# kv13arm/mujoco_rl_manipulate_unknown_objects

Hardware: AMD Instinct MI355X
Metric: env-steps/sec (whole node), acorn_env 4096 envs/GPU (higher is better)
Workload: dtype f32

## Files before the change

### mujoco_rl_manipulate_unknown_objects_amd/csrc/grip_render.hip

```cpp
#include <hip/hip_runtime.h>
#include <cstdio>
#include <cstdlib>
#include <algorithm>
#include "grip_device.h"
#include <atomic>

int grip_fail(const char *msg);
static int launch_status(const char *what) {
    hipError_t e = hipGetLastError();
    if (e == hipSuccess) return 0;
    char buf[256]; snprintf(buf, sizeof buf, "%s: %s", what, hipGetErrorString(e));
    return grip_fail(buf);
}

#define RW 64
#define RH 64
#define RTHREADS 1024
#define RPIX (RW * RH)

struct Frames { float p[6][3]; float R[6][9]; float cam_o[3]; float cam_R[9]; };

__device__ static void compute_frames(const DevModel &m, const float *qpos, int n, int e, int half, Frames &f) {
    float q[14];
    for (int i = 0; i < 14; i++) q[i] = ld_word(qpos, (size_t)i * n + e, half);
    V3 pe = v3(m.ee_pos0[0] + q[0], m.ee_pos0[1] + q[1], m.ee_pos0[2] + q[2]);
    float sr = sinf(q[3]), cr = cosf(q[3]), sy = sinf(q[4]), cy = cosf(q[4]);
    M3 Re;
    Re.m[0] = cy; Re.m[1] = -sy; Re.m[2] = 0.f; Re.m[3] = cr * sy; Re.m[4] = cr * cy; Re.m[5] = -sr; Re.m[6] = sr * sy; Re.m[7] = sr * cy; Re.m[8] = cr;
    auto put = [&](int g, V3 p, const M3 &R) { f.p[g][0] = p.x; f.p[g][1] = p.y; f.p[g][2] = p.z; for (int i = 0; i < 9; i++) f.R[g][i] = R.m[i]; };
    V3 pb = pe + mulv(Re, ldv(m.base_pos)); M3 Rb = mulm(Re, ldm(m.base_R));
    put(0, pb, Rb);
    for (int s = 0; s < 2; s++) {
        V3 pk = pb + mulv(Rb, ldv(m.kn_pos[s])); M3 Rk0 = mulm(Rb, ldm(m.kn_R[s]));
        float sq = sinf(q[5 + s]), cq = cosf(q[5 + s]);
        M3 Ry; Ry.m[0] = cq; Ry.m[1] = 0; Ry.m[2] = sq; Ry.m[3] = 0; Ry.m[4] = 1; Ry.m[5] = 0; Ry.m[6] = -sq; Ry.m[7] = 0; Ry.m[8] = cq;
        M3 Rk = mulm(Rk0, Ry);
        put(1 + 2 * s, pk, Rk);
        put(2 + 2 * s, pk + mulv(Rk, ldv(m.fin_pos[s])), mulm(Rk, ldm(m.fin_R[s])));
    }
    float qn = rsqrtf(q[10] * q[10] + q[11] * q[11] + q[12] * q[12] + q[13] * q[13]);
    put(5, v3(q[7], q[8], q[9]), quat_mat(q[10] * qn, q[11] * qn, q[12] * qn, q[13] * qn));
    V3 co = pe + mulv(Re, ldv(m.cam_pos)); M3 Rc = mulm(Re, ldm(m.cam_R));
    f.cam_o[0] = co.x; f.cam_o[1] = co.y; f.cam_o[2] = co.z;
    for (int i = 0; i < 9; i++) f.cam_R[i] = Rc.m[i];
}


__device__ __forceinline__ void frame_role(const DevModel &m, const float *qpos, int n, int e, int half, int role, Frames &f) {
    auto Q = [&](int i) { return ld_word(qpos, (size_t)i * n + e, half); };
    V3 P; M3 R;
    if (role == 5) {
        const float q0 = Q(10), q1 = Q(11), q2 = Q(12), q3 = Q(13);
        const float qn = rsqrtf(q0 * q0 + q1 * q1 + q2 * q2 + q3 * q3);
        P = v3(Q(7), Q(8), Q(9)); R = quat_mat(q0 * qn, q1 * qn, q2 * qn, q3 * qn);
    } else {
        const V3 pe = v3(m.ee_pos0[0] + Q(0), m.ee_pos0[1] + Q(1), m.ee_pos0[2] + Q(2));
        const float q3 = Q(3), q4 = Q(4);
        const float sr = sinf(q3), cr = cosf(q3), sy = sinf(q4), cy = cosf(q4);
        M3 Re;
        Re.m[0] = cy; Re.m[1] = -sy; Re.m[2] = 0.f; Re.m[3] = cr * sy; Re.m[4] = cr * cy; Re.m[5] = -sr; Re.m[6] = sr * sy; Re.m[7] = sr * cy; Re.m[8] = cr;
        if (role == 6) { P = pe + mulv(Re, ldv(m.cam_pos)); R = mulm(Re, ldm(m.cam_R)); }
        else {
            P = pe + mulv(Re, ldv(m.base_pos)); R = mulm(Re, ldm(m.base_R));
            if (role >= 1) {
                const int s = role >= 3 ? 1 : 0;
                const V3 pk = P + mulv(R, ldv(m.kn_pos[s])); const M3 Rk0 = mulm(R, ldm(m.kn_R[s]));
                const float qk = Q(5 + s);
                const float sq = sinf(qk), cq = cosf(qk);
                M3 Ry; Ry.m[0] = cq; Ry.m[1] = 0; Ry.m[2] = sq; Ry.m[3] = 0; Ry.m[4] = 1; Ry.m[5] = 0; Ry.m[6] = -sq; Ry.m[7] = 0; Ry.m[8] = cq;
                P = pk; R = mulm(Rk0, Ry);
                if (role == 2 || role == 4) { const V3 pf = P + mulv(R, ldv(m.fin_pos[s])); const M3 Rf = mulm(R, ldm(m.fin_R[s])); P = pf; R = Rf; }
            }
        }
    }
    float *op = role == 6 ? f.cam_o : f.p[role], *oR = role == 6 ? f.cam_R : f.R[role];
    op[0] = P.x; op[1] = P.y; op[2] = P.z;
#pragma unroll
    for (int i = 0; i < 9; i++) oR[i] = R.m[i];
}

__device__ static uint8_t to_u8(float v) { v *= 255.f; v = fminf(fmaxf(v, 0.f), 255.f); return (uint8_t)v; }

__device__ __forceinline__ void lit_colour(const DevModel &m, int geom, float b0, float b1, float b2, V3 P, V3 N, V3 co, float &c0, float &c1, float &c2) {
    const float spec = m.geom_material[geom][0], shin = 128.f * m.geom_material[geom][1];
    const V3 V = normalized(co - P);
    float diff = m.geom_material[geom][2] + m.headlight[0], sp = 0.f;
    {   const float nv = dot(N, V);
        if (nv > 0.f) { diff += m.headlight[1] * nv; sp += m.headlight[2] * __powf(nv, shin); } }
#pragma unroll
    for (int l = 0; l < 2; l++) {
        const V3 ld = normalized(ldv(m.light_dir[l]));
        V3 L = -ld; float spot = 1.f;
        if (!m.light_directional[l]) {
            L = normalized(ldv(m.light_pos[l]) - P);
            const float c = -dot(L, ld);
            spot = c > m.light_params[l][3] ? __powf(c, m.light_params[l][4]) : 0.f;
        }
        diff += m.light_params[l][2];
        const float nl = dot(N, L);
        if (nl > 0.f && spot > 0.f) {
            diff += spot * m.light_params[l][0] * nl;
            const float nh = fmaxf(dot(N, normalized(L + V)), 0.f);
            sp += spot * m.light_params[l][1] * __powf(nh, shin);
        }
    }
    c0 = b0 * diff + spec * sp; c1 = b1 * diff + spec * sp; c2 = b2 * diff + spec * sp;
}
// ... 267 lines not shown
#pragma unroll
    for (int q = 0; q < TPX; q++) { float d = best[q] - dmin; if (d <= 1.0f) { lsum += d; lcnt++; } }
    red[tid] = lsum; redi[tid] = lcnt; __syncthreads();
    for (int s = RTHREADS / 2; s > 0; s >>= 1) { if (tid < s) { red[tid] += red[tid + s]; redi[tid] += redi[tid + s]; } __syncthreads(); }
    float scale = 2.0f * (red[0] / (float)redi[0]);
    if (cfg.full_observation) {
        unsigned db[TPX];
#pragma unroll
        for (int q = 0; q < TPX; q++) {
            float v = (best[q] - dmin) / scale; v = fminf(fmaxf(v, 0.f), 1.f);
            float p = 255.0f * v;
            db[q] = (p != p) ? 0u : (unsigned)(uint8_t)p;
        }
#pragma unroll
        for (int r = 0; r < TW; r++) put2(3, r, db[2 * r], db[2 * r + 1]);
    }
    __syncthreads();
    if (tid == 0) {
        const int pg_ = GPTR(const int, pad_grasp)[e], pp_ = GPTR(const int, pad_pher)[e];
        img[(nch - 1) * RPIX] = (uint8_t)pg_; img[(nch - 1) * RPIX + 1] = (uint8_t)pp_;
    }
    __syncthreads();
    const uint4 *src = reinterpret_cast<const uint4 *>(img);
    for (int i = tid; i < nch * RPIX / 16; i += RTHREADS) {
        const uint4 v = src[i];
        if (o) reinterpret_cast<uint4 *>(o)[i] = v;
        if (o2) reinterpret_cast<uint4 *>(o2)[i] = v;
    }
}

#ifndef RS_SMALL
#define RS_SMALL 16
#endif
#ifndef RS_WAVES
#define RS_WAVES 8
#endif
#ifndef RS_FACES
#define RS_FACES 255
#endif
#ifndef RS_QUAD
#define RS_QUAD 1
#endif
#define RS_LDS_BUDGET (80 * 1024 - 34 * 1024)
#define RS_DYN_BYTES(nverts, edges, items) ((size_t)(((nverts) * 3 + 3) / 4 * 4) * 4 + (size_t)RS_FACES * 32 + (size_t)(edges) * 16 + (size_t)(items) * 2)
struct __align__(16) RsFace { float4 P; int ebase, k, id, pad; };
static_assert(!RS_QUAD || RS_FACES <= 255, "a quad item holds the face record in 8 bits, and 0xffff must stay free");

__device__ __forceinline__ void rs_claim(unsigned long long *zb, int pix, float t, int id) {
    atomicMin(zb + pix, ((unsigned long long)__float_as_uint(t) << 32) | (unsigned)id);
}

__device__ __forceinline__ void observe_body_raster(const DevModel &m, const DevConfig &cfg, const float *qpos, const int *pad_grasp, const int *pad_pher,
                                                    int n, int e, uint8_t *obs, uint8_t *obs2, const long long *row2, int nverts_max, const int RS_EDGES, const int RS_ITEMS) {
    __shared__ Frames fr;
    __shared__ float gmx[GN_GEOM][12];
    __shared__ int gnum[GN_GEOM];
    __shared__ int nfaces, nedges, nitems;
    __shared__ __align__(16) unsigned char pool[8 * RPIX];
    extern __shared__ float4 rs_dyn[];
    unsigned long long *zb = reinterpret_cast<unsigned long long *>(pool);
    uint8_t *img = pool; float *red = reinterpret_cast<float *>(pool + 5 * RPIX); int *redi = reinterpret_cast<int *>(pool + 6 * RPIX);
    float *cv = reinterpret_cast<float *>(rs_dyn);
    RsFace *frec = reinterpret_cast<RsFace *>(cv + (nverts_max * 3 + 3) / 4 * 4);
    float4 *en = reinterpret_cast<float4 *>(frec + RS_FACES);
    unsigned short *items = reinterpret_cast<unsigned short *>(en + RS_EDGES);
    const int tid = threadIdx.x;
    const int nvert_all = m.hull_vadr[GN_HULL - 1] + m.hull_vnum[GN_HULL - 1], nplane_all = m.hull_padr[GN_HULL - 1] + m.hull_pnum[GN_HULL - 1];
    auto hull_of_vertex = [&](int i) { int g = 1; for (int h = 2; h < GN_GEOM; h++) g = i >= m.hull_vadr[h - 1] ? h : g; return g; };
    auto hull_of_plane = [&](int i) { int g = 1; for (int h = 2; h < GN_GEOM; h++) g = i >= m.hull_padr[h - 1] ? h : g; return g; };
    constexpr int VPT = 2;
    float4 vearly[VPT];
    {   const float4 *vb = reinterpret_cast<const float4 *>(m.hull_blob);
#pragma unroll
        for (int k = 0; k < VPT; k++) { const int i = tid + k * RTHREADS; vearly[k] = i < nvert_all ? vb[i] : make_float4(0.f, 0.f, 0.f, 0.f); }
    }
    if (tid < 7) frame_role(m, qpos, n, e, cfg.state_half, tid, fr);
    if (tid == 0) { nfaces = 0; nedges = 0; nitems = 0; }
    for (int i = tid; i < RPIX; i += RTHREADS) zb[i] = ~0ull;
    for (int i = tid; i < RS_ITEMS; i += RTHREADS) items[i] = 0xffffu;
    __syncthreads();
    if (tid >= 1 && tid < GN_GEOM) {
        const int g = tid;
        V3 co = ldv(fr.cam_o); M3 Rc = ldm(fr.cam_R);
        V3 p = ldv(fr.p[g - 1]); M3 R = ldm(fr.R[g - 1]);
        V3 c = multv(Rc, p + mulv(R, ldv(m.geom_center[g])) - co);
        float r = m.geom_rbound[g];
        M3 Mx = mulm(M3{{R.m[0], R.m[3], R.m[6], R.m[1], R.m[4], R.m[7], R.m[2], R.m[5], R.m[8]}}, Rc);
        V3 ol = multv(R, co - p);
#pragma unroll
        for (int i = 0; i < 9; i++) gmx[g][i] = Mx.m[i];
        gmx[g][9] = ol.x; gmx[g][10] = ol.y; gmx[g][11] = ol.z;
        bool vis = c.z - r < 0.f;
        if (vis) {
            const float th = tanf(0.5f * m.cam_fovy * 0.017453292519943295f) * 1.0001f;
            unsigned out = 0x1fu;
            for (int k = 0; k < 8; k++) {
                const V3 q = multv(Mx, v3(m.hull_aabb[g - 1][(k & 1) ? 3 : 0] - ol.x, m.hull_aabb[g - 1][(k & 2) ? 4 : 1] - ol.y, m.hull_aabb[g - 1][(k & 4) ? 5 : 2] - ol.z));
                const float d = -q.z * th + 1e-6f;
                unsigned o_ = 0u;
                o_ |= q.z > -m.znear ? 1u : 0u; o_ |= q.x > d ? 2u : 0u; o_ |= q.x < -d ? 4u : 0u; o_ |= q.y > d ? 8u : 0u; o_ |= q.y < -d ? 16u : 0u;
                out &= o_;
            }
            vis = out == 0u;
        }
        gnum[g] = vis ? m.hull_pnum[g - 1] : 0;
    }
    __syncthreads();
    const float tanh_ = tanf(0.5f * m.cam_fovy * 0.017453292519943295f);
    auto ray_x = [&](int px) { return (2.0f * (px + 0.5f) / RW - 1.0f) * tanh_; };
    auto ray_y = [&](int py) { return (1.0f - 2.0f * (py + 0.5f) / RH) * tanh_; };
    {
        const float4 *vb = reinterpret_cast<const float4 *>(m.hull_blob);
        auto to_camera = [&](int i, float4 v) {
            const int g = hull_of_vertex(i);
            const int *gn = gnum; asm volatile("" : "+v"(gn));
            if (!gn[g]) return;
            const M3 Mx = ldm(gmx[g]);
            const V3 c = multv(Mx, v3(v.x - gmx[g][9], v.y - gmx[g][10], v.z - gmx[g][11]));
            cv[3 * i] = c.x; cv[3 * i + 1] = c.y; cv[3 * i + 2] = c.z;
        };
#pragma unroll
        for (int k = 0; k < VPT; k++) if (tid + k * RTHREADS < nvert_all) to_camera(tid + k * RTHREADS, vearly[k]);
        for (int i = tid + VPT * RTHREADS; i < nvert_all; i += RTHREADS) to_camera(i, vb[i]);
    }
    __syncthreads();
#ifndef RS_STOP
#define RS_STOP 0
#endif
    if (RS_STOP != 1) {
        for (int i = tid; i < nplane_all; i += RTHREADS) {
            const int jg = nplane_all - 1 - i, g = hull_of_plane(jg), j = jg - m.hull_padr[g - 1];
            {   const int *gn = gnum; asm volatile("" : "+v"(gn)); if (!gn[g]) continue; }
            const int l0 = m.hull_ladr[jg], K = m.hull_ladr[jg + 1] - l0;
            if (K < 3) continue;
            const float *pl = m.hull_planes + 4 * jg;
            const V3 nn = v3(pl[0], pl[1], pl[2]);
            const M3 Mx = ldm(gmx[g]);
            const V3 A = multv(Mx, nn);
            const float B = pl[3] - dot(nn, v3(gmx[g][9], gmx[g][10], gmx[g][11]));
            if (!(B < 0.f)) continue;
            const float *cvg = cv + 3 * m.hull_vadr[g - 1];
            const int *lp = m.hull_loops + l0;
            int id4[4]; V3 v4[4];
            float xmin = 3.0e38f, xmax = -3.0e38f, ymin = 3.0e38f, ymax = -3.0e38f;
            const float zn = -m.znear;
            auto take = [&](float x, float y, float z) {
                const float iz = rcp(-z), px = x * iz, py = y * iz;
                xmin = fminf(xmin, px); xmax = fmaxf(xmax, px); ymin = fminf(ymin, py); ymax = fmaxf(ymax, py);
            };
            auto corner = [&](V3 prev, V3 cur) {
                const bool ic = cur.z <= zn, ip = prev.z <= zn;
                if (ic) take(cur.x, cur.y, cur.z);
                if (ic != ip) { const float s_ = (zn - prev.z) * rcp(cur.z - prev.z); take(fmaf(s_, cur.x - prev.x, prev.x), fmaf(s_, cur.y - prev.y, prev.y), zn); }
            };
            auto vert = [&](int id) { return v3(cvg[3 * id], cvg[3 * id + 1], cvg[3 * id + 2]); };
#pragma unroll
            for (int k = 0; k < 4; k++) { id4[k] = lp[k < K ? k : 0]; v4[k] = vert(id4[k]); }
            V3 prev = K == 3 ? v4[2] : (K == 4 ? v4[3] : vert(lp[K - 1]));
#pragma unroll
            for (int k = 0; k < 4; k++) if (k < K) { corner(prev, v4[k]); prev = v4[k]; }
            for (int k = 4; k < K; k++) { const V3 c = vert(lp[k]); corner(prev, c); prev = c; }
            if (!(xmin <= xmax)) continue;
            int x0, x1, y0, y1;
            {
                const float sx = 0.5f * RW / tanh_, sy = 0.5f * RH / tanh_;
                const float fx0 = xmin * sx + 0.5f * RW - 0.5f, fx1 = xmax * sx + 0.5f * RW - 0.5f;
                const float fy0 = 0.5f * RH - ymax * sy - 0.5f, fy1 = 0.5f * RH - ymin * sy - 0.5f;
                if (fx1 < -0.01f || fy1 < -0.01f || fx0 > RW - 0.99f || fy0 > RH - 0.99f) continue;
                x0 = (int)ceilf(fmaxf(fx0 - 0.01f, 0.f)); x1 = (int)floorf(fminf(fx1 + 0.01f, RW - 1.f));
                y0 = (int)ceilf(fmaxf(fy0 - 0.01f, 0.f)); y1 = (int)floorf(fminf(fy1 + 0.01f, RH - 1.f));
                if (x0 > x1 || y0 > y1) continue;
            }
            const int idw = (g << 16) | j;
            const int area = (x1 - x0 + 1) * (y1 - y0 + 1);
            auto edge = [&](int ia, V3 a, int ib, V3 b) { const bool sw = ia > ib; const V3 c = cross(sw ? b : a, sw ? a : b); return sw ? -c : c; };
            if (K <= 4 && area <= RS_SMALL) {
                V3 ne[4];
#pragma unroll
                for (int k = 0; k < 4; k++) {
                    const int kn = (k + 1 < K) ? k + 1 : 0;
                    ne[k] = k < K ? edge(id4[k], v4[k], id4[kn], v4[kn]) : v3(0.f, 0.f, 0.f);
                }
                int px = x0, py = y0;
                for (int q = 0; q < area; q++) {
                    const float x = ray_x(px), y = ray_y(py);
                    bool in = true;
#pragma unroll
                    for (int k = 0; k < 4; k++) in &= !(fmaf(ne[k].x, x, fmaf(ne[k].y, y, -ne[k].z)) > 0.f);
                    const float den = fmaf(A.y, y, fmaf(A.x, x, -A.z));
                    const float t = B * rcp(den);
                    if (in && den < 0.f && t > 0.f && t > m.znear) rs_claim(zb, py * RW + px, t, idw);
                    if (++px > x1) { px = x0; ++py; }
                }
                continue;
            }
            constexpr int TS = RS_QUAD ? 2 : 3, TB = RS_QUAD ? 8 : 6;
            const int tx0 = x0 >> TS, tx1 = x1 >> TS, ty0 = y0 >> TS, ty1 = y1 >> TS, ntile = (tx1 - tx0 + 1) * (ty1 - ty0 + 1);
            int fi = atomicAdd(&nfaces, 1), eb = -1, ib = -1;
            if (fi < RS_FACES) { eb = atomicAdd(&nedges, K); if (eb + K <= RS_EDGES) { ib = atomicAdd(&nitems, ntile); if (ib + ntile > RS_ITEMS) ib = -1; } }
            if (ib >= 0) {
                RsFace f; f.P = make_float4(A.x, A.y, A.z, B); f.ebase = eb; f.k = K; f.id = idw; f.pad = 0;
                frec[fi] = f;
                int ia = lp[0]; V3 a = v3(cvg[3 * ia], cvg[3 * ia + 1], cvg[3 * ia + 2]);
                const int i0 = ia; const V3 a0 = a;
                for (int k = 0; k < K; k++) {
                    const int ib2 = k + 1 < K ? lp[k + 1] : i0;
                    const V3 b = k + 1 < K ? v3(cvg[3 * ib2], cvg[3 * ib2 + 1], cvg[3 * ib2 + 2]) : a0;
                    const V3 c = edge(ia, a, ib2, b);
                    en[eb + k] = make_float4(c.x, c.y, c.z, 0.f);
                    ia = ib2; a = b;
                }
                int w = ib;
                for (int ty = ty0; ty <= ty1; ty++) for (int tx = tx0; tx <= tx1; tx++) items[w++] = (unsigned short)((fi << TB) | ((ty << (6 - TS)) + tx));
                continue;
            }
            for (int py = y0; py <= y1; py++) for (int px = x0; px <= x1; px++) {
                const float x = ray_x(px), y = ray_y(py);
                bool in = true;
                int ia = lp[0]; V3 a = v3(cvg[3 * ia], cvg[3 * ia + 1], cvg[3 * ia + 2]);
                const int i0 = ia; const V3 a0 = a;
                for (int k = 0; k < K; k++) {
                    const int ib2 = k + 1 < K ? lp[k + 1] : i0;
                    const V3 b = k + 1 < K ? v3(cvg[3 * ib2], cvg[3 * ib2 + 1], cvg[3 * ib2 + 2]) : a0;
                    const V3 c = edge(ia, a, ib2, b);
                    in &= !(fmaf(c.x, x, fmaf(c.y, y, -c.z)) > 0.f);
                    ia = ib2; a = b;
                }
                const float den = fmaf(A.y, y, fmaf(A.x, x, -A.z));
                const float t = B * rcp(den);
                if (in && den < 0.f && t > 0.f && t > m.znear) rs_claim(zb, py * RW + px, t, idw);
            }
        }
    }
    __syncthreads();
    if (RS_STOP != 1 && RS_STOP != 2) {
        const int ni = min(nitems, RS_ITEMS), wv = tid >> 6, ln = tid & 63;
#if RS_QUAD
        auto fetch = [&](int it0, unsigned &item, RsFace &f) {
            const int it = it0 + (ln >> 4);
            item = it < ni ? (unsigned)items[it] : 0xffffu;
            f = frec[item != 0xffffu ? (item >> 8) : 0];
        };
        unsigned item, item_n = 0xffffu; RsFace f, f_n;
        fetch(4 * wv, item, f);
        for (int it0 = 4 * wv; it0 < ni; it0 += 4 * (RTHREADS / 64)) {
            if (it0 + 4 * (RTHREADS / 64) < ni) fetch(it0 + 4 * (RTHREADS / 64), item_n, f_n);
            const bool live = item != 0xffffu;
            const int K = live ? f.k : 0;
            const int quad = item & 255, px = (quad & 15) * 4 + (ln & 3), py = (quad >> 4) * 4 + ((ln >> 2) & 3);
            const float x = ray_x(px), y = ray_y(py);
            bool in = live;
            const float4 *ep = en + f.ebase;
            for (int k0 = 0; __any(k0 < K); k0 += 4) {
                float4 c[4];
#pragma unroll
                for (int j = 0; j < 4; j++) c[j] = ep[max(min(k0 + j, K - 1), 0)];
#pragma unroll
                for (int j = 0; j < 4; j++) in &= !(fmaf(c[j].x, x, fmaf(c[j].y, y, -c[j].z)) > 0.f);
            }
            const float den = fmaf(f.P.y, y, fmaf(f.P.x, x, -f.P.z));
            const float t = f.P.w * rcp(den);
            if (in && den < 0.f && t > 0.f && t > m.znear) rs_claim(zb, py * RW + px, t, f.id);
            item = item_n; f = f_n; item_n = 0xffffu;
        }
#else
        for (int it = wv; it < ni; it += RTHREADS / 64) {
            const unsigned item = __builtin_amdgcn_readfirstlane((unsigned)items[it]);
            if (item == 0xffffu) continue;
            RsFace f = frec[item >> 6];
            f.k = __builtin_amdgcn_readfirstlane(f.k); f.ebase = __builtin_amdgcn_readfirstlane(f.ebase);
            const int tile = item & 63, px = (tile & 7) * 8 + (ln & 7), py = (tile >> 3) * 8 + (ln >> 3);
            const float x = ray_x(px), y = ray_y(py);
            bool in = true;
            const float4 *ep = en + f.ebase;
            for (int k = 0; k < f.k; k++) { const float4 c = ep[k]; in &= !(fmaf(c.x, x, fmaf(c.y, y, -c.z)) > 0.f); }
            const float den = fmaf(f.P.y, y, fmaf(f.P.x, x, -f.P.z));
            const float t = f.P.w * rcp(den);
            if (in && den < 0.f && t > 0.f && t > m.znear) rs_claim(zb, py * RW + px, t, f.id);
        }
#endif
    }
    __syncthreads();
    const Frames *frl = &fr;
    asm volatile("" : "+v"(frl));
    const int nch = cfg.full_observation ? 5 : 4;
    uint8_t *o = obs ? obs + (size_t)blockIdx.x * nch * RPIX : nullptr;
    uint8_t *o2 = obs2 ? obs2 + (size_t)(row2[0] + blockIdx.x) * nch * RPIX : nullptr;
    constexpr int WPR = RW / (8 * TW);
    const int w = tid >> 6, l = tid & 63;
    const int tx = (l & 7) + 8 * (w % WPR), ty = (l >> 3) + 8 * (w / WPR);
    float xs[TW], ys[TW];
#pragma unroll
    for (int a = 0; a < TW; a++) { xs[a] = ray_x(TW * tx + a); ys[a] = ray_y(TW * ty + a); }
    float best[TPX]; int hitent[TPX];
#pragma unroll
    for (int q = 0; q < TPX; q++) {
        float x = xs[q % TW], y = ys[q / TW];
        float dz = frl->cam_R[6] * x + frl->cam_R[7] * y - frl->cam_R[8];
        best[q] = m.zfar; hitent[q] = -1;
        if (dz < 0.f) { float t = -frl->cam_o[2] / dz; if (t > m.znear && t < best[q]) { best[q] = t; hitent[q] = 0; } }
        const unsigned long long z = zb[(TW * ty + q / TW) * RW + TW * tx + q % TW];
        const float th = __uint_as_float((unsigned)(z >> 32));
        if (z != ~0ull && th < best[q]) { best[q] = th; hitent[q] = (int)(unsigned)z; }
    }
    __syncthreads();
    asm volatile("" : "+v"(frl));
    const V3 co = ldv(frl->cam_o); const M3 Rc = ldm(frl->cam_R);
    float lmin = 3.0e38f;
#pragma unroll
    for (int q = 0; q < TPX; q++) {
        const float x = xs[q % TW], y = ys[q / TW];
        const V3 dir = mulv(Rc, v3(x, y, -1.f));
        const int hit = hitent[q] < 0 ? -1 : (hitent[q] >> 16);
        float c0, c1, c2;
        if (hit < 0) {
            V3 dn = normalized(dir); float f = 0.5f * (dn.z + 1.0f);
            c0 = m.sky_rgb[3] + f * (m.sky_rgb[0] - m.sky_rgb[3]); c1 = m.sky_rgb[4] + f * (m.sky_rgb[1] - m.sky_rgb[4]); c2 = m.sky_rgb[5] + f * (m.sky_rgb[2] - m.sky_rgb[5]);
        } else {
            float b0, b1, b2; V3 nrm = v3(0, 0, 1);
            const V3 Pw = co + dir * best[q];
            if (hit == 0) {
                int cx = (int)floorf(Pw.x * 8.0f), cy = (int)floorf(Pw.y * 8.0f);
                int off = ((cx + cy) & 1) ? 3 : 0;
                b0 = m.floor_rgb[off]; b1 = m.floor_rgb[off + 1]; b2 = m.floor_rgb[off + 2];
            } else {
                b0 = m.geom_rgba[hit][0]; b1 = m.geom_rgba[hit][1]; b2 = m.geom_rgba[hit][2];
                const float *pl = m.hull_planes + 4 * (m.hull_padr[hit - 1] + (hitent[q] & 0xffff));
                const V3 A = multv(ldm(gmx[hit]), v3(pl[0], pl[1], pl[2]));
                nrm = normalized(mulv(Rc, A));
            }
#if defined(RS_SKIP) && (RS_SKIP & 1)
            c0 = b0 * nrm.z; c1 = b1 * Pw.x; c2 = b2;
#else
            lit_colour(m, hit, b0, b1, b2, Pw, nrm, co, c0, c1, c2);
#endif
        }
        {   const int px = (TW * ty + q / TW) * RW + TW * tx + q % TW;
            img[px] = to_u8(c0); img[RPIX + px] = to_u8(c1); img[2 * RPIX + px] = to_u8(c2); }
        lmin = fminf(lmin, best[q]);
        __builtin_amdgcn_sched_barrier(0);
    }
    auto put2 = [&](int ch, int r, unsigned lo, unsigned hi) {
        const int px = (TW * ty + r) * RW + TW * tx;
        *reinterpret_cast<uint16_t *>(img + ch * RPIX + px) = (uint16_t)(lo | (hi << 8));
    };
#pragma unroll
    for (int r = 0; r < TW; r++) put2(nch - 1, r, 0u, 0u);
#if defined(RS_SKIP) && (RS_SKIP & 2)
    float dmin = lmin; red[0] = 1.f; redi[0] = 1;
#else
    red[tid] = lmin; __syncthreads();
    for (int s = RTHREADS / 2; s > 0; s >>= 1) { if (tid < s) red[tid] = fminf(red[tid], red[tid + s]); __syncthreads(); }
    float dmin = red[0]; __syncthreads();
    float lsum = 0.f; int lcnt = 0;
#pragma unroll
    for (int q = 0; q < TPX; q++) { float d = best[q] - dmin; if (d <= 1.0f) { lsum += d; lcnt++; } }
    red[tid] = lsum; redi[tid] = lcnt; __syncthreads();
    for (int s = RTHREADS / 2; s > 0; s >>= 1) { if (tid < s) { red[tid] += red[tid + s]; redi[tid] += redi[tid + s]; } __syncthreads(); }
#endif
    float scale = 2.0f * (red[0] / (float)redi[0]);
    if (cfg.full_observation) {
        unsigned db[TPX];
#pragma unroll
        for (int q = 0; q < TPX; q++) {
            float v = (best[q] - dmin) / scale; v = fminf(fmaxf(v, 0.f), 1.f);
            float p = 255.0f * v;
            db[q] = (p != p) ? 0u : (unsigned)(uint8_t)p;
        }
#pragma unroll
        for (int r = 0; r < TW; r++) put2(3, r, db[2 * r], db[2 * r + 1]);
    }
    __syncthreads();
    if (tid == 0) {
        const int pg_ = GPTR(const int, pad_grasp)[e], pp_ = GPTR(const int, pad_pher)[e];
        img[(nch - 1) * RPIX] = (uint8_t)pg_; img[(nch - 1) * RPIX + 1] = (uint8_t)pp_;
    }
    __syncthreads();
#ifdef RS_DEBUG_COUNTS
    if (tid == 0) { int *d = reinterpret_cast<int *>(img); d[0] = nfaces; d[1] = nedges; d[2] = nitems; d[3] = gnum[1] + gnum[2] + gnum[3] + gnum[4] + gnum[5] + gnum[6]; }
    __syncthreads();
#endif
    const uint4 *src = reinterpret_cast<const uint4 *>(img);
    for (int i = tid; i < nch * RPIX / 16; i += RTHREADS) {
        const uint4 v = src[i];
        if (o) reinterpret_cast<uint4 *>(o)[i] = v;
        if (o2) reinterpret_cast<uint4 *>(o2)[i] = v;
    }
}

__global__ void __launch_bounds__(RTHREADS, 8) k_observe_rays(const RenderGroup *__restrict__ groups, int ngroups, const int *list, const int *count,
                                                           uint8_t *obs, uint8_t *obs2, const long long *row2) {
    if (list && count && (int)blockIdx.x >= *count) return;
    const int ge = list ? list[blockIdx.x] : (int)blockIdx.x;
    if (ge < 0) return;
    int g = 0;
    for (int i = 1; i < ngroups; i++) g = ge >= groups[i].env0 ? i : g;
    const RenderGroup &rg = groups[g];
    const DevConfig cfg = rg.cfg;
    observe_body(rg.m, cfg, rg.qpos, rg.pad_grasp, rg.pad_pher, rg.n, ge - rg.env0, obs, obs2, row2);
}

__global__ void __launch_bounds__(RTHREADS, RS_WAVES) k_observe(const RenderGroup *__restrict__ groups, int ngroups, const int *list, const int *count,
                                                      uint8_t *obs, uint8_t *obs2, const long long *row2, int nverts_max, int edges_cap, int items_cap) {
    if (list && count && (int)blockIdx.x >= *count) return;
    const int ge = list ? list[blockIdx.x] : (int)blockIdx.x;
    if (ge < 0) return;
    int g = 0;
    for (int i = 1; i < ngroups; i++) g = ge >= groups[i].env0 ? i : g;
    const RenderGroup &rg = groups[g];
    const DevConfig cfg = rg.cfg;
    observe_body_raster(rg.m, cfg, rg.qpos, rg.pad_grasp, rg.pad_pher, rg.n, ge - rg.env0, obs, obs2, row2, nverts_max, edges_cap, items_cap);
}

static bool observe_by_rays() {
    static const bool v = [] { const char *e = getenv("GRIP_OBSERVE_RAYS"); return e && e[0] == '1'; }();
    return v;
}
#define RS_MAX_VERTS 4096

extern "C" int grip_render_launch(const RenderGroup *groups_dev, int ngroups, const int *list, const int *count, int nblocks, int nplanes_max, int nverts_max,
                                  uint8_t *obs, uint8_t *obs2, const long long *row2, hipStream_t s) {
    const bool rays = observe_by_rays();
    if (!rays && (nverts_max < 1 || nverts_max > RS_MAX_VERTS)) return grip_fail("grip_render_launch: the model's hulls have more vertices than the observation kernel's LDS table holds (RS_MAX_VERTS)");
    {
        static std::atomic<unsigned long long> attr_set_mask{0ULL};
        int dev = 0;
        if (hipGetDevice(&dev) != hipSuccess) return -1;
        const unsigned long long bit = 1ULL << (dev & 63);
        if (!(attr_set_mask.load(std::memory_order_acquire) & bit)) {
            if (hipFuncSetAttribute((const void *)k_observe_rays, hipFuncAttributeMaxDynamicSharedMemorySize, (int)((RMAXPL + NBOX * GN_HULL) * sizeof(float4))) != hipSuccess) return -1;
            if (hipFuncSetAttribute((const void *)k_observe, hipFuncAttributeMaxDynamicSharedMemorySize, (int)RS_DYN_BYTES(RS_MAX_VERTS, 1024, 8192)) != hipSuccess) return -1;
            attr_set_mask.fetch_or(bit, std::memory_order_release);
        }
    }
    if (rays)
        hipLaunchKernelGGL(k_observe_rays, dim3(nblocks), dim3(RTHREADS), (size_t)(nplanes_max + NBOX * GN_HULL) * sizeof(float4), s, groups_dev, ngroups, list, count, obs, obs2, row2);
    else {
        const long long left = (long long)RS_LDS_BUDGET - (long long)RS_DYN_BYTES(nverts_max, 0, 0);
        const int edges_cap = left >= 1024 * 16 + 2048 * 2 ? 1024 : 512;
        const int items_cap = (int)std::min<long long>(8192, std::max<long long>(1024, (left - edges_cap * 16) / 2)) & ~7;
        hipLaunchKernelGGL(k_observe, dim3(nblocks), dim3(RTHREADS), RS_DYN_BYTES(nverts_max, edges_cap, items_cap), s, groups_dev, ngroups, list, count, obs, obs2, row2, nverts_max,
                           edges_cap, items_cap);
    }
    return launch_status("grip_render_launch");
}

__global__ void __launch_bounds__(256) k_render_camera(const RenderGroup *__restrict__ groups, int e, const float *cam, float fovy_deg, int w, int h,
                                                       uint8_t *rgb, float *depth) {
    __shared__ Frames fr;
    const RenderGroup &rg = groups[0];
    const DevModel &m = rg.m;
    if (threadIdx.x == 0) {
        compute_frames(m, rg.qpos, rg.n, e, rg.cfg.state_half, fr);
        if (cam) { for (int i = 0; i < 3; i++) fr.cam_o[i] = cam[i]; for (int i = 0; i < 9; i++) fr.cam_R[i] = cam[3 + i]; }
    }
    __syncthreads();
    const int px = blockIdx.x * blockDim.x + threadIdx.x;
    if (px >= w * h) return;
    const int i = px / w, j = px % w;
    const V3 co = ldv(fr.cam_o); const M3 Rc = ldm(fr.cam_R);
    const float th = tanf(0.5f * fovy_deg * 0.017453292519943295f), tw = th * (float)w / (float)h;
    const float x = (2.0f * (j + 0.5f) / w - 1.0f) * tw, y = (1.0f - 2.0f * (i + 0.5f) / h) * th;
    const V3 dir = mulv(Rc, v3(x, y, -1.f));
    float best = m.zfar; int hit = -1; V3 nrm = v3(0, 0, 1);
    if (dir.z < 0.f) { float t = -co.z / dir.z; if (t > m.znear && t < best) { best = t; hit = 0; } }
    for (int g = 1; g < GN_GEOM; g++) {
        const V3 p = ldv(fr.p[g - 1]); const M3 R = ldm(fr.R[g - 1]);
        const V3 ol = multv(R, co - p), dl = multv(R, dir);
        const float *pl = m.hull_planes + 4 * m.hull_padr[g - 1];
        float tin = -3.0e38f, tout = 3.0e38f; int ent = -1;
        for (int k = 0; k < m.hull_pnum[g - 1]; k++) {
            const V3 nn = v3(pl[4 * k], pl[4 * k + 1], pl[4 * k + 2]);
            const float den = dot(nn, dl), num = pl[4 * k + 3] - dot(nn, ol);
            if (den < 0.f) { const float t = num / den; if (t > tin) { tin = t; ent = k; } }
// ... 95 lines not shown
```

Measured before the change: 178,100.

## Shrink raster observation LDS and block size to fit three envs per CU

The raster observation kernel drops from 1024 to 512 threads per block, with each thread covering two pixel tiles. The per-vertex camera-space LDS table is removed, so vertices are transformed on the fly from global memory. Each geometry thread computes its own frames, which drops a barrier. The face, edge and item caps become fixed and smaller so that LDS use allows three blocks per CU. The tree reductions are replaced by wave shuffles plus a cross-wave sum. The risks are redundant vertex transforms, more global loads, and more faces falling back to the slow per-pixel path when the smaller tables overflow.

```diff
diff --git a/mujoco_rl_manipulate_unknown_objects_amd/csrc/grip_render.hip b/mujoco_rl_manipulate_unknown_objects_amd/csrc/grip_render.hip
--- a/mujoco_rl_manipulate_unknown_objects_amd/csrc/grip_render.hip
+++ b/mujoco_rl_manipulate_unknown_objects_amd/csrc/grip_render.hip
@@ -46,9 +46,8 @@
 }
 
 
-__device__ __forceinline__ void frame_role(const DevModel &m, const float *qpos, int n, int e, int half, int role, Frames &f) {
+__device__ __forceinline__ void frame_role_pr(const DevModel &m, const float *qpos, int n, int e, int half, int role, V3 &P, M3 &R) {
     auto Q = [&](int i) { return ld_word(qpos, (size_t)i * n + e, half); };
-    V3 P; M3 R;
     if (role == 5) {
         const float q0 = Q(10), q1 = Q(11), q2 = Q(12), q3 = Q(13);
         const float qn = rsqrtf(q0 * q0 + q1 * q1 + q2 * q2 + q3 * q3);
@@ -73,6 +72,10 @@
             }
         }
     }
+}
+__device__ __forceinline__ void frame_role(const DevModel &m, const float *qpos, int n, int e, int half, int role, Frames &f) {
+    V3 P; M3 R;
+    frame_role_pr(m, qpos, n, e, half, role, P, R);
     float *op = role == 6 ? f.cam_o : f.p[role], *oR = role == 6 ? f.cam_R : f.R[role];
     op[0] = P.x; op[1] = P.y; op[2] = P.z;
 #pragma unroll
@@ -406,57 +409,93 @@
 #ifndef RS_SMALL
 #define RS_SMALL 16
 #endif
+#ifndef RS_THREADS
+#define RS_THREADS 512
+#endif
+#define RS_NW (RS_THREADS / 64)
 #ifndef RS_WAVES
-#define RS_WAVES 8
+#define RS_WAVES 6
 #endif
 #ifndef RS_FACES
-#define RS_FACES 255
+#define RS_FACES 240
 #endif
 #ifndef RS_QUAD
 #define RS_QUAD 1
 #endif
-#define RS_LDS_BUDGET (80 * 1024 - 34 * 1024)
-#define RS_DYN_BYTES(nverts, edges, items) ((size_t)(((nverts) * 3 + 3) / 4 * 4) * 4 + (size_t)RS_FACES * 32 + (size_t)(edges) * 16 + (size_t)(items) * 2)
+#define RS_EDGES_CAP 640
+#define RS_ITEMS_CAP 1024
+#define RS_DYN_BYTES(faces, edges, items) ((size_t)(faces) * 32 + (size_t)(edges) * 16 + (size_t)(((items) + 7) & ~7) * 2)
 struct __align__(16) RsFace { float4 P; int ebase, k, id, pad; };
 static_assert(!RS_QUAD || RS_FACES <= 255, "a quad item holds the face record in 8 bits, and 0xffff must stay free");
+static_assert(RS_THREADS == 512, "the resolve / shade mapping and the reductions' association are written for 8 waves");
+static_assert(32 * 1024 + 512 + RS_DYN_BYTES(RS_FACES, RS_EDGES_CAP, RS_ITEMS_CAP) <= 52 * 1024, "three envs per CU, whatever the granule of the LDS allocation up to 2 KB");
+
+__device__ unsigned long long g_rs_fallbacks;
+extern "C" int grip_debug_observe_fallbacks(unsigned long long *out) {
+    if (hipDeviceSynchronize() != hipSuccess) return -1;
+    return hipMemcpyFromSymbol(out, HIP_SYMBOL(g_rs_fallbacks), sizeof(unsigned long long)) == hipSuccess ? 0 : -1;
+}
+
+#ifdef RS_STAMPS
+#define RS_NPHASE 16
+__device__ unsigned long long g_rs_stamps[RS_NPHASE + 1][2];
+#define RS_T0() unsigned long long rs_t = __builtin_amdgcn_s_memtime()
+#define RS_MARK(i, j) do { __builtin_amdgcn_sched_barrier(0); const unsigned long long n_ = __builtin_amdgcn_s_memtime(); __builtin_amdgcn_s_waitcnt(0xC07F); \
+                           if ((threadIdx.x & 63) == 0) atomicAdd(&g_rs_stamps[i][j], n_ - rs_t); rs_t = n_; __builtin_amdgcn_sched_barrier(0); } while (0)
+#define RS_WORK(i) RS_MARK(i, 0)
+#define RS_WAIT(i) RS_MARK(i, 1)
+#define RS_DONE() do { if ((threadIdx.x & 63) == 0) atomicAdd(&g_rs_stamps[RS_NPHASE][0], 1ull); } while (0)
+extern "C" const char *grip_debug_rs_phase_names() {
+    return "init, frames, hull visibility (6 threads) | face set-up + small faces | item pass (quads) | resolve against the floor | shading (lit_colour) + wave minimum | sum partials, wave count | cross-wave sum + depth bytes | store to HBM";
+}
+extern "C" int grip_debug_rs_stamps(unsigned long long *out, int reset) {
+    if (hipDeviceSynchronize() != hipSuccess) return -1;
+    if (out && hipMemcpyFromSymbol(out, HIP_SYMBOL(g_rs_stamps), sizeof(unsigned long long) * (RS_NPHASE + 1) * 2) != hipSuccess) return -1;
+    if (reset) { static const unsigned long long zero[RS_NPHASE + 1][2] = {}; if (hipMemcpyToSymbol(HIP_SYMBOL(g_rs_stamps), zero, sizeof zero) != hipSuccess) return -1; }
+    return 0;
+}
+#else
+#define RS_T0() do { } while (0)
+#define RS_WORK(i) do { } while (0)
+#define RS_WAIT(i) do { } while (0)
+#define RS_DONE() do { } while (0)
+#endif
 
 __device__ __forceinline__ void rs_claim(unsigned long long *zb, int pix, float t, int id) {
     atomicMin(zb + pix, ((unsigned long long)__float_as_uint(t) << 32) | (unsigned)id);
 }
 
 __device__ __forceinline__ void observe_body_raster(const DevModel &m, const DevConfig &cfg, const float *qpos, const int *pad_grasp, const int *pad_pher,
-                                                    int n, int e, uint8_t *obs, uint8_t *obs2, const long long *row2, int nverts_max, const int RS_EDGES, const int RS_ITEMS) {
-    __shared__ Frames fr;
+                                                    int n, int e, uint8_t *obs, uint8_t *obs2, const long long *row2, const int RS_NFACE, const int RS_EDGES, const int RS_ITEMS) {
+    __shared__ float cam[12];
     __shared__ float gmx[GN_GEOM][12];
     __shared__ int gnum[GN_GEOM];
     __shared__ int nfaces, nedges, nitems;
+    __shared__ float wmin[RS_NW]; __shared__ int wcnt[RS_NW];
     __shared__ __align__(16) unsigned char pool[8 * RPIX];
     extern __shared__ float4 rs_dyn[];
     unsigned long long *zb = reinterpret_cast<unsigned long long *>(pool);
-    uint8_t *img = pool; float *red = reinterpret_cast<float *>(pool + 5 * RPIX); int *redi = reinterpret_cast<int *>(pool + 6 * RPIX);
-    float *cv = reinterpret_cast<float *>(rs_dyn);
-    RsFace *frec = reinterpret_cast<RsFace *>(cv + (nverts_max * 3 + 3) / 4 * 4);
-    float4 *en = reinterpret_cast<float4 *>(frec + RS_FACES);
+    uint8_t *img = pool; float *red = reinterpret_cast<float *>(pool + 5 * RPIX);
+    RsFace *frec = reinterpret_cast<RsFace *>(rs_dyn);
+    float4 *en = reinterpret_cast<float4 *>(frec + RS_NFACE);
     unsigned short *items = reinterpret_cast<unsigned short *>(en + RS_EDGES);
     const int tid = threadIdx.x;
-    const int nvert_all = m.hull_vadr[GN_HULL - 1] + m.hull_vnum[GN_HULL - 1], nplane_all = m.hull_padr[GN_HULL - 1] + m.hull_pnum[GN_HULL - 1];
-    auto hull_of_vertex = [&](int i) { int g = 1; for (int h = 2; h < GN_GEOM; h++) g = i >= m.hull_vadr[h - 1] ? h : g; return g; };
+    RS_T0();
+    const int nplane_all = m.hull_padr[GN_HULL - 1] + m.hull_pnum[GN_HULL - 1];
     auto hull_of_plane = [&](int i) { int g = 1; for (int h = 2; h < GN_GEOM; h++) g = i >= m.hull_padr[h - 1] ? h : g; return g; };
-    constexpr int VPT = 2;
-    float4 vearly[VPT];
-    {   const float4 *vb = reinterpret_cast<const float4 *>(m.hull_blob);
-#pragma unroll
-        for (int k = 0; k < VPT; k++) { const int i = tid + k * RTHREADS; vearly[k] = i < nvert_all ? vb[i] : make_float4(0.f, 0.f, 0.f, 0.f); }
-    }
-    if (tid < 7) frame_role(m, qpos, n, e, cfg.state_half, tid, fr);
     if (tid == 0) { nfaces = 0; nedges = 0; nitems = 0; }
-    for (int i = tid; i < RPIX; i += RTHREADS) zb[i] = ~0ull;
-    for (int i = tid; i < RS_ITEMS; i += RTHREADS) items[i] = 0xffffu;
-    __syncthreads();
+    for (int i = tid; i < RPIX; i += RS_THREADS) zb[i] = ~0ull;
+    for (int i = tid; i < RS_ITEMS; i += RS_THREADS) items[i] = 0xffffu;
     if (tid >= 1 && tid < GN_GEOM) {
         const int g = tid;
-        V3 co = ldv(fr.cam_o); M3 Rc = ldm(fr.cam_R);
-        V3 p = ldv(fr.p[g - 1]); M3 R = ldm(fr.R[g - 1]);
+        V3 co, p; M3 Rc, R;
+        frame_role_pr(m, qpos, n, e, cfg.state_half, 6, co, Rc);
+        frame_role_pr(m, qpos, n, e, cfg.state_half, g - 1, p, R);
+        if (g == 1) {
+            cam[0] = co.x; cam[1] = co.y; cam[2] = co.z;
+#pragma unroll
+            for (int i = 0; i < 9; i++) cam[3 + i] = Rc.m[i];
+        }
         V3 c = multv(Rc, p + mulv(R, ldv(m.geom_center[g])) - co);
         float r = m.geom_rbound[g];
         M3 Mx = mulm(M3{{R.m[0], R.m[3], R.m[6], R.m[1], R.m[4], R.m[7], R.m[2], R.m[5], R.m[8]}}, Rc);
@@ -479,30 +518,15 @@
         }
         gnum[g] = vis ? m.hull_pnum[g - 1] : 0;
     }
-    __syncthreads();
+    RS_WORK(0); __syncthreads(); RS_WAIT(0);
     const float tanh_ = tanf(0.5f * m.cam_fovy * 0.017453292519943295f);
     auto ray_x = [&](int px) { return (2.0f * (px + 0.5f) / RW - 1.0f) * tanh_; };
     auto ray_y = [&](int py) { return (1.0f - 2.0f * (py + 0.5f) / RH) * tanh_; };
-    {
-        const float4 *vb = reinterpret_cast<const float4 *>(m.hull_blob);
-        auto to_camera = [&](int i, float4 v) {
-            const int g = hull_of_vertex(i);
-            const int *gn = gnum; asm volatile("" : "+v"(gn));
-            if (!gn[g]) return;
-            const M3 Mx = ldm(gmx[g]);
-            const V3 c = multv(Mx, v3(v.x - gmx[g][9], v.y - gmx[g][10], v.z - gmx[g][11]));
-            cv[3 * i] = c.x; cv[3 * i + 1] = c.y; cv[3 * i + 2] = c.z;
-        };
-#pragma unroll
-        for (int k = 0; k < VPT; k++) if (tid + k * RTHREADS < nvert_all) to_camera(tid + k * RTHREADS, vearly[k]);
-        for (int i = tid + VPT * RTHREADS; i < nvert_all; i += RTHREADS) to_camera(i, vb[i]);
-    }
-    __syncthreads();
 #ifndef RS_STOP
 #define RS_STOP 0
 #endif
     if (RS_STOP != 1) {
-        for (int i = tid; i < nplane_all; i += RTHREADS) {
+        for (int i = tid; i < nplane_all; i += RS_THREADS) {
             const int jg = nplane_all - 1 - i, g = hull_of_plane(jg), j = jg - m.hull_padr[g - 1];
             {   const int *gn = gnum; asm volatile("" : "+v"(gn)); if (!gn[g]) continue; }
             const int l0 = m.hull_ladr[jg], K = m.hull_ladr[jg + 1] - l0;
@@ -513,8 +537,9 @@
             const V3 A = multv(Mx, nn);
             const float B = pl[3] - dot(nn, v3(gmx[g][9], gmx[g][10], gmx[g][11]));
             if (!(B < 0.f)) continue;
-            const float *cvg = cv + 3 * m.hull_vadr[g - 1];
             const int *lp = m.hull_loops + l0;
+            const float4 *vbg = reinterpret_cast<const float4 *>(m.hull_blob) + m.hull_vadr[g - 1];
+            auto vert = [&](int id) { const float4 v = vbg[id]; return multv(Mx, v3(v.x - gmx[g][9], v.y - gmx[g][10], v.z - gmx[g][11])); };
             int id4[4]; V3 v4[4];
             float xmin = 3.0e38f, xmax = -3.0e38f, ymin = 3.0e38f, ymax = -3.0e38f;
             const float zn = -m.znear;
@@ -527,7 +552,6 @@
                 if (ic) take(cur.x, cur.y, cur.z);
                 if (ic != ip) { const float s_ = (zn - prev.z) * rcp(cur.z - prev.z); take(fmaf(s_, cur.x - prev.x, prev.x), fmaf(s_, cur.y - prev.y, prev.y), zn); }
             };
-            auto vert = [&](int id) { return v3(cvg[3 * id], cvg[3 * id + 1], cvg[3 * id + 2]); };
 #pragma unroll
             for (int k = 0; k < 4; k++) { id4[k] = lp[k < K ? k : 0]; v4[k] = vert(id4[k]); }
             V3 prev = K == 3 ? v4[2] : (K == 4 ? v4[3] : vert(lp[K - 1]));
@@ -571,15 +595,15 @@
             constexpr int TS = RS_QUAD ? 2 : 3, TB = RS_QUAD ? 8 : 6;
             const int tx0 = x0 >> TS, tx1 = x1 >> TS, ty0 = y0 >> TS, ty1 = y1 >> TS, ntile = (tx1 - tx0 + 1) * (ty1 - ty0 + 1);
             int fi = atomicAdd(&nfaces, 1), eb = -1, ib = -1;
-            if (fi < RS_FACES) { eb = atomicAdd(&nedges, K); if (eb + K <= RS_EDGES) { ib = atomicAdd(&nitems, ntile); if (ib + ntile > RS_ITEMS) ib = -1; } }
+            if (fi < RS_NFACE) { eb = atomicAdd(&nedges, K); if (eb + K <= RS_EDGES) { ib = atomicAdd(&nitems, ntile); if (ib + ntile > RS_ITEMS) ib = -1; } }
             if (ib >= 0) {
                 RsFace f; f.P = make_float4(A.x, A.y, A.z, B); f.ebase = eb; f.k = K; f.id = idw; f.pad = 0;
                 frec[fi] = f;
-                int ia = lp[0]; V3 a = v3(cvg[3 * ia], cvg[3 * ia + 1], cvg[3 * ia + 2]);
+                int ia = lp[0]; V3 a = vert(ia);
                 const int i0 = ia; const V3 a0 = a;
                 for (int k = 0; k < K; k++) {
                     const int ib2 = k + 1 < K ? lp[k + 1] : i0;
-                    const V3 b = k + 1 < K ? v3(cvg[3 * ib2], cvg[3 * ib2 + 1], cvg[3 * ib2 + 2]) : a0;
+                    const V3 b = k + 1 < K ? vert(ib2) : a0;
                     const V3 c = edge(ia, a, ib2, b);
                     en[eb + k] = make_float4(c.x, c.y, c.z, 0.f);
                     ia = ib2; a = b;
@@ -588,14 +612,15 @@
                 for (int ty = ty0; ty <= ty1; ty++) for (int tx = tx0; tx <= tx1; tx++) items[w++] = (unsigned short)((fi << TB) | ((ty << (6 - TS)) + tx));
                 continue;
             }
+            atomicAdd(&g_rs_fallbacks, 1ull);
             for (int py = y0; py <= y1; py++) for (int px = x0; px <= x1; px++) {
                 const float x = ray_x(px), y = ray_y(py);
                 bool in = true;
-                int ia = lp[0]; V3 a = v3(cvg[3 * ia], cvg[3 * ia + 1], cvg[3 * ia + 2]);
+                int ia = lp[0]; V3 a = vert(ia);
                 const int i0 = ia; const V3 a0 = a;
                 for (int k = 0; k < K; k++) {
                     const int ib2 = k + 1 < K ? lp[k + 1] : i0;
-                    const V3 b = k + 1 < K ? v3(cvg[3 * ib2], cvg[3 * ib2 + 1], cvg[3 * ib2 + 2]) : a0;
+                    const V3 b = k + 1 < K ? vert(ib2) : a0;
                     const V3 c = edge(ia, a, ib2, b);
                     in &= !(fmaf(c.x, x, fmaf(c.y, y, -c.z)) > 0.f);
                     ia = ib2; a = b;
@@ -606,7 +631,7 @@
             }
         }
     }
-    __syncthreads();
+    RS_WORK(1); __syncthreads(); RS_WAIT(1);
     if (RS_STOP != 1 && RS_STOP != 2) {
         const int ni = min(nitems, RS_ITEMS), wv = tid >> 6, ln = tid & 63;
 #if RS_QUAD
@@ -617,8 +642,8 @@
         };
         unsigned item, item_n = 0xffffu; RsFace f, f_n;
         fetch(4 * wv, item, f);
-        for (int it0 = 4 * wv; it0 < ni; it0 += 4 * (RTHREADS / 64)) {
-            if (it0 + 4 * (RTHREADS / 64) < ni) fetch(it0 + 4 * (RTHREADS / 64), item_n, f_n);
+        for (int it0 = 4 * wv; it0 < ni; it0 += 4 * RS_NW) {
+            if (it0 + 4 * RS_NW < ni) fetch(it0 + 4 * RS_NW, item_n, f_n);
             const bool live = item != 0xffffu;
             const int K = live ? f.k : 0;
             const int quad = item & 255, px = (quad & 15) * 4 + (ln & 3), py = (quad >> 4) * 4 + ((ln >> 2) & 3);
@@ -638,7 +663,7 @@
             item = item_n; f = f_n; item_n = 0xffffu;
         }
 #else
-        for (int it = wv; it < ni; it += RTHREADS / 64) {
+        for (int it = wv; it < ni; it += RS_NW) {
             const unsigned item = __builtin_amdgcn_readfirstlane((unsigned)items[it]);
             if (item == 0xffffu) continue;
             RsFace f = frec[item >> 6];
@@ -654,36 +679,40 @@
         }
 #endif
     }
-    __syncthreads();
-    const Frames *frl = &fr;
-    asm volatile("" : "+v"(frl));
+    RS_WORK(2); __syncthreads(); RS_WAIT(2);
+    const float *cml = cam;
+    asm volatile("" : "+v"(cml));
     const int nch = cfg.full_observation ? 5 : 4;
     uint8_t *o = obs ? obs + (size_t)blockIdx.x * nch * RPIX : nullptr;
     uint8_t *o2 = obs2 ? obs2 + (size_t)(row2[0] + blockIdx.x) * nch * RPIX : nullptr;
-    constexpr int WPR = RW / (8 * TW);
+    constexpr int WPR = RW / (8 * TW), NT = 2, NPX = NT * TPX, TYS = RH / TW / NT;
     const int w = tid >> 6, l = tid & 63;
     const int tx = (l & 7) + 8 * (w % WPR), ty = (l >> 3) + 8 * (w / WPR);
-    float xs[TW], ys[TW];
-#pragma unroll
-    for (int a = 0; a < TW; a++) { xs[a] = ray_x(TW * tx + a); ys[a] = ray_y(TW * ty + a); }
-    float best[TPX]; int hitent[TPX];
-#pragma unroll
-    for (int q = 0; q < TPX; q++) {
-        float x = xs[q % TW], y = ys[q / TW];
-        float dz = frl->cam_R[6] * x + frl->cam_R[7] * y - frl->cam_R[8];
+    auto pix_x = [&](int q) { return TW * tx + q % TW; };
+    auto pix_y = [&](int q) { return TW * (ty + TYS * (q / TPX)) + (q % TPX) / TW; };
+    float xs[TW], ys[NT * TW];
+#pragma unroll
+    for (int a = 0; a < TW; a++) xs[a] = ray_x(TW * tx + a);
+#pragma unroll
+    for (int a = 0; a < NT * TW; a++) ys[a] = ray_y(TW * (ty + TYS * (a / TW)) + a % TW);
+    float best[NPX]; int hitent[NPX];
+#pragma unroll
+    for (int q = 0; q < NPX; q++) {
+        float x = xs[q % TW], y = ys[TW * (q / TPX) + (q % TPX) / TW];
+        float dz = cml[3 + 6] * x + cml[3 + 7] * y - cml[3 + 8];
         best[q] = m.zfar; hitent[q] = -1;
-        if (dz < 0.f) { float t = -frl->cam_o[2] / dz; if (t > m.znear && t < best[q]) { best[q] = t; hitent[q] = 0; } }
-        const unsigned long long z = zb[(TW * ty + q / TW) * RW + TW * tx + q % TW];
+        if (dz < 0.f) { float t = -cml[2] / dz; if (t > m.znear && t < best[q]) { best[q] = t; hitent[q] = 0; } }
+        const unsigned long long z = zb[pix_y(q) * RW + pix_x(q)];
         const float th = __uint_as_float((unsigned)(z >> 32));
         if (z != ~0ull && th < best[q]) { best[q] = th; hitent[q] = (int)(unsigned)z; }
     }
-    __syncthreads();
-    asm volatile("" : "+v"(frl));
-    const V3 co = ldv(frl->cam_o); const M3 Rc = ldm(frl->cam_R);
+    RS_WORK(3); __syncthreads(); RS_WAIT(3);
+    asm volatile("" : "+v"(cml));
+    const V3 co = ldv(cml); const M3 Rc = ldm(cml + 3);
     float lmin = 3.0e38f;
 #pragma unroll
-    for (int q = 0; q < TPX; q++) {
-        const float x = xs[q % TW], y = ys[q / TW];
+    for (int q = 0; q < NPX; q++) {
+        const float x = xs[q % TW], y = ys[TW * (q / TPX) + (q % TPX) / TW];
         const V3 dir = mulv(Rc, v3(x, y, -1.f));
         const int hit = hitent[q] < 0 ? -1 : (hitent[q] >> 16);
         float c0, c1, c2;
@@ -709,57 +738,84 @@
             lit_colour(m, hit, b0, b1, b2, Pw, nrm, co, c0, c1, c2);
 #endif
         }
-        {   const int px = (TW * ty + q / TW) * RW + TW * tx + q % TW;
+        {   const int px = pix_y(q) * RW + pix_x(q);
             img[px] = to_u8(c0); img[RPIX + px] = to_u8(c1); img[2 * RPIX + px] = to_u8(c2); }
         lmin = fminf(lmin, best[q]);
         __builtin_amdgcn_sched_barrier(0);
     }
     auto put2 = [&](int ch, int r, unsigned lo, unsigned hi) {
-        const int px = (TW * ty + r) * RW + TW * tx;
+        const int px = (TW * (ty + TYS * (r / TW)) + r % TW) * RW + TW * tx;
         *reinterpret_cast<uint16_t *>(img + ch * RPIX + px) = (uint16_t)(lo | (hi << 8));
     };
-#pragma unroll
-    for (int r = 0; r < TW; r++) put2(nch - 1, r, 0u, 0u);
+    {   unsigned p0 = 0u, p1 = 0u;
+        if (tid == 0) { p0 = (unsigned)(uint8_t)GPTR(const int, pad_grasp)[e]; p1 = (unsigned)(uint8_t)GPTR(const int, pad_pher)[e]; }
+#pragma unroll
+        for (int r = 0; r < NT * TW; r++) put2(nch - 1, r, r == 0 ? p0 : 0u, r == 0 ? p1 : 0u);
+    }
 #if defined(RS_SKIP) && (RS_SKIP & 2)
-    float dmin = lmin; red[0] = 1.f; redi[0] = 1;
+    float dmin = lmin; const float tsum = 1.f; const int tcnt = 1;
 #else
-    red[tid] = lmin; __syncthreads();
-    for (int s = RTHREADS / 2; s > 0; s >>= 1) { if (tid < s) red[tid] = fminf(red[tid], red[tid + s]); __syncthreads(); }
-    float dmin = red[0]; __syncthreads();
-    float lsum = 0.f; int lcnt = 0;
-#pragma unroll
-    for (int q = 0; q < TPX; q++) { float d = best[q] - dmin; if (d <= 1.0f) { lsum += d; lcnt++; } }
-    red[tid] = lsum; redi[tid] = lcnt; __syncthreads();
-    for (int s = RTHREADS / 2; s > 0; s >>= 1) { if (tid < s) { red[tid] += red[tid + s]; redi[tid] += redi[tid + s]; } __syncthreads(); }
+#pragma unroll
+    for (int s = 32; s > 0; s >>= 1) lmin = fminf(lmin, __shfl_xor(lmin, s));
+    if (l == 0) wmin[w] = lmin;
+    RS_WORK(4); __syncthreads(); RS_WAIT(4);
+    float dmin = wmin[0];
+#pragma unroll
+    for (int k = 1; k < RS_NW; k++) dmin = fminf(dmin, wmin[k]);
+    float tsum; int tcnt;
+    {   float part[NT]; int lcnt = 0;
+#pragma unroll
+        for (int h = 0; h < NT; h++) {
+            float lsum = 0.f;
+#pragma unroll
+            for (int q = 0; q < TPX; q++) { float d = best[h * TPX + q] - dmin; if (d <= 1.0f) { lsum += d; lcnt++; } }
+            part[h] = lsum;
+        }
+        red[tid] = part[0] + part[1];
+#pragma unroll
+        for (int s = 32; s > 0; s >>= 1) lcnt += __shfl_xor(lcnt, s);
+        if (l == 0) wcnt[w] = lcnt;
+        RS_WORK(5); __syncthreads(); RS_WAIT(5);
+        float a[RS_NW];
+#pragma unroll
+        for (int k = 0; k < RS_NW; k++) a[k] = red[64 * k + l];
+#pragma unroll
+        for (int k = 0; k < 4; k++) a[k] = a[k] + a[k + 4];
+#pragma unroll
+        for (int k = 0; k < 2; k++) a[k] = a[k] + a[k + 2];
+        float v = a[0] + a[1];
+#pragma unroll
+        for (int s = 32; s > 0; s >>= 1) v = v + __shfl_down(v, s);
+        tsum = __shfl(v, 0);
+        tcnt = 0;
+#pragma unroll
+        for (int k = 0; k < RS_NW; k++) tcnt += wcnt[k];
+    }
 #endif
-    float scale = 2.0f * (red[0] / (float)redi[0]);
+    float scale = 2.0f * (tsum / (float)tcnt);
     if (cfg.full_observation) {
-        unsigned db[TPX];
-#pragma unroll
-        for (int q = 0; q < TPX; q++) {
+        unsigned db[NPX];
+#pragma unroll
+        for (int q = 0; q < NPX; q++) {
             float v = (best[q] - dmin) / scale; v = fminf(fmaxf(v, 0.f), 1.f);
             float p = 255.0f * v;
             db[q] = (p != p) ? 0u : (unsigned)(uint8_t)p;
         }
 #pragma unroll
-        for (int r = 0; r < TW; r++) put2(3, r, db[2 * r], db[2 * r + 1]);
-    }
-    __syncthreads();
-    if (tid == 0) {
-        const int pg_ = GPTR(const int, pad_grasp)[e], pp_ = GPTR(const int, pad_pher)[e];
-        img[(nch - 1) * RPIX] = (uint8_t)pg_; img[(nch - 1) * RPIX + 1] = (uint8_t)pp_;
-    }
-    __syncthreads();
+        for (int r = 0; r < NT * TW; r++) put2(3, r, db[2 * r], db[2 * r + 1]);
+    }
+    RS_WORK(6); __syncthreads(); RS_WAIT(6);
 #ifdef RS_DEBUG_COUNTS
     if (tid == 0) { int *d = reinterpret_cast<int *>(img); d[0] = nfaces; d[1] = nedges; d[2] = nitems; d[3] = gnum[1] + gnum[2] + gnum[3] + gnum[4] + gnum[5] + gnum[6]; }
     __syncthreads();
 #endif
     const uint4 *src = reinterpret_cast<const uint4 *>(img);
-    for (int i = tid; i < nch * RPIX / 16; i += RTHREADS) {
+    for (int i = tid; i < nch * RPIX / 16; i += RS_THREADS) {
         const uint4 v = src[i];
         if (o) reinterpret_cast<uint4 *>(o)[i] = v;
         if (o2) reinterpret_cast<uint4 *>(o2)[i] = v;
     }
+    RS_WORK(7); RS_DONE();
 }
 
 __global__ void __launch_bounds__(RTHREADS, 8) k_observe_rays(const RenderGroup *__restrict__ groups, int ngroups, const int *list, const int *count,
@@ -774,8 +830,8 @@
     observe_body(rg.m, cfg, rg.qpos, rg.pad_grasp, rg.pad_pher, rg.n, ge - rg.env0, obs, obs2, row2);
 }
 
-__global__ void __launch_bounds__(RTHREADS, RS_WAVES) k_observe(const RenderGroup *__restrict__ groups, int ngroups, const int *list, const int *count,
-                                                      uint8_t *obs, uint8_t *obs2, const long long *row2, int nverts_max, int edges_cap, int items_cap) {
+__global__ void __launch_bounds__(RS_THREADS, RS_WAVES) k_observe(const RenderGroup *__restrict__ groups, int ngroups, const int *list, const int *count,
+                                                      uint8_t *obs, uint8_t *obs2, const long long *row2, int faces_cap, int edges_cap, int items_cap) {
     if (list && count && (int)blockIdx.x >= *count) return;
     const int ge = list ? list[blockIdx.x] : (int)blockIdx.x;
     if (ge < 0) return;
@@ -783,19 +839,22 @@
     for (int i = 1; i < ngroups; i++) g = ge >= groups[i].env0 ? i : g;
     const RenderGroup &rg = groups[g];
     const DevConfig cfg = rg.cfg;
-    observe_body_raster(rg.m, cfg, rg.qpos, rg.pad_grasp, rg.pad_pher, rg.n, ge - rg.env0, obs, obs2, row2, nverts_max, edges_cap, items_cap);
+    observe_body_raster(rg.m, cfg, rg.qpos, rg.pad_grasp, rg.pad_pher, rg.n, ge - rg.env0, obs, obs2, row2, faces_cap, edges_cap, items_cap);
 }
 
 static bool observe_by_rays() {
     static const bool v = [] { const char *e = getenv("GRIP_OBSERVE_RAYS"); return e && e[0] == '1'; }();
     return v;
 }
-#define RS_MAX_VERTS 4096
+static bool observe_small_tables() {
+    static const bool v = [] { const char *e = getenv("GRIP_OBSERVE_SMALL_TABLES"); return e && e[0] == '1'; }();
+    return v;
+}
 
 extern "C" int grip_render_launch(const RenderGroup *groups_dev, int ngroups, const int *list, const int *count, int nblocks, int nplanes_max, int nverts_max,
                                   uint8_t *obs, uint8_t *obs2, const long long *row2, hipStream_t s) {
     const bool rays = observe_by_rays();
-    if (!rays && (nverts_max < 1 || nverts_max > RS_MAX_VERTS)) return grip_fail("grip_render_launch: the model's hulls have more vertices than the observation kernel's LDS table holds (RS_MAX_VERTS)");
+    (void)nverts_max;
     {
         static std::atomic<unsigned long long> attr_set_mask{0ULL};
         int dev = 0;
@@ -803,17 +862,16 @@
         const unsigned long long bit = 1ULL << (dev & 63);
         if (!(attr_set_mask.load(std::memory_order_acquire) & bit)) {
             if (hipFuncSetAttribute((const void *)k_observe_rays, hipFuncAttributeMaxDynamicSharedMemorySize, (int)((RMAXPL + NBOX * GN_HULL) * sizeof(float4))) != hipSuccess) return -1;
-            if (hipFuncSetAttribute((const void *)k_observe, hipFuncAttributeMaxDynamicSharedMemorySize, (int)RS_DYN_BYTES(RS_MAX_VERTS, 1024, 8192)) != hipSuccess) return -1;
+            if (hipFuncSetAttribute((const void *)k_observe, hipFuncAttributeMaxDynamicSharedMemorySize, (int)RS_DYN_BYTES(RS_FACES, RS_EDGES_CAP, RS_ITEMS_CAP)) != hipSuccess) return -1;
             attr_set_mask.fetch_or(bit, std::memory_order_release);
         }
     }
     if (rays)
         hipLaunchKernelGGL(k_observe_rays, dim3(nblocks), dim3(RTHREADS), (size_t)(nplanes_max + NBOX * GN_HULL) * sizeof(float4), s, groups_dev, ngroups, list, count, obs, obs2, row2);
     else {
-        const long long left = (long long)RS_LDS_BUDGET - (long long)RS_DYN_BYTES(nverts_max, 0, 0);
-        const int edges_cap = left >= 1024 * 16 + 2048 * 2 ? 1024 : 512;
-        const int items_cap = (int)std::min<long long>(8192, std::max<long long>(1024, (left - edges_cap * 16) / 2)) & ~7;
-        hipLaunchKernelGGL(k_observe, dim3(nblocks), dim3(RTHREADS), RS_DYN_BYTES(nverts_max, edges_cap, items_cap), s, groups_dev, ngroups, list, count, obs, obs2, row2, nverts_max,
+        const bool small = observe_small_tables();
+        const int faces_cap = small ? 4 : RS_FACES, edges_cap = small ? 16 : RS_EDGES_CAP, items_cap = small ? 16 : RS_ITEMS_CAP;
+        hipLaunchKernelGGL(k_observe, dim3(nblocks), dim3(RS_THREADS), RS_DYN_BYTES(faces_cap, edges_cap, items_cap), s, groups_dev, ngroups, list, count, obs, obs2, row2, faces_cap,
                            edges_cap, items_cap);
     }
     return launch_status("grip_render_launch");
```

After: 149,500. 0.839x the previous value.
